# Maaz77/Head-Pose-Estimation-Model

Hardware: AMD Instinct MI355X
Metric: images/sec (train+infer) on 96×96 feature maps; yaw/pitch/roll MAE vs ref (higher is better)
Workload: dtype fp32; 1 GPU; Model-96 create_model(num_filters=360, dropout=0, l2=0.1) training, legacy Adam lr 2.8e-4, 96x96 feature maps (configs[3] per GPU: 512 images per rank); global_batch=512, per_gpu_batch=512, positions_per_image=9216, channels=96, parallelism=dp1

## Files before the change

### head-pose-estimation-model_amd/csrc/hpe_mlp2.hip

```cpp
#include <hip/hip_runtime.h>
#include <stdint.h>
#include <stdlib.h>
#include <type_traits>

#include "hpe_common.h"
#include "hpe_dev.h"

#ifdef MLP2_BIG
#define MLP2_NS mlp2_big
#define MLP2_BIG_OBJ 1
#else
#define MLP2_NS mlp2_small
#define MLP2_BIG_OBJ 0
#endif
#define MLP2_BIG_ROWS (1 << 15)
namespace MLP2_NS {

#define MLP2_MAXW 12
#ifndef MLP2_BAR1_SKIP
#define MLP2_BAR1_SKIP 1
#endif
#ifndef MLP2_W88
#define MLP2_W88 2
#endif
// ... 134 lines not shown
}
__device__ __forceinline__ constexpr int a1_row(int g) { return 68 * (g ^ ((g >> 1) & 4)); }
#define MLP2_X_LIMIT (65520.f / SPLIT_C)
template <int KH>
__device__ __forceinline__ bool presplit_tile(const float* xs, _Float16* xf, int tid, int NT) {
  bool out = false;
  for (int i = tid; i < 32 * 12; i += NT) {
    const int r = i / 12, rem = i - r * 12, h = rem >= 6 ? 1 : 0, m0 = 8 * (rem - 6 * h);
    const float* s = xs + r * MLP2_XS + KH * h + m0;
    const f32x4 z = {0.f, 0.f, 0.f, 0.f};
    const f32x4 a = *(const f32x4*)(s), b = m0 + 4 < KH ? *(const f32x4*)(s + 4) : z;
    const f32x8 v = {a.x, a.y, a.z, a.w, b.x, b.y, b.z, b.w};
#pragma unroll
    for (int j = 0; j < 8; ++j) out |= !(fabsf(v[j]) < MLP2_X_LIMIT);
    const SplitD d8 = split_d8(v);
    _Float16* d = xf + img_row(r) * MLP2_FS + 48 * h + m0;
    *(h8*)(d) = d8.ch;
    *(h8*)(d + 32 * MLP2_FS) = d8.cl;
    *(h8*)(d + 64 * MLP2_FS) = d8.h;
  }
  return out;
}

__device__ __forceinline__ SplitW split_w8_mix(f32x8 v) {
  SplitW r;
  r.h = __builtin_convertvector(v, h8);
  f32x8 lo;
#pragma unroll
  for (int j = 0; j < 8; ++j) lo[j] = __builtin_fmaf((float)r.h[j], -SPLIT_C, v[j] * SPLIT_C);
  r.cl = __builtin_convertvector(lo, h8);
  return r;
}

template <int KH, int ACT1, bool DROP, int NWM, bool SPLIT, bool CONTIG = false>
__global__ void __launch_bounds__(NWM * 64) __attribute__((amdgpu_waves_per_eu(NWM == MLP2_MAXW || ACT1 < 0 ? 1 : MLP2_W88, 8))) mlp2_kernel(Args args) {
  static_assert(!CONTIG || (SPLIT && NWM == MLP2_MAXW), "CONTIG is an instantiation of the pre-split kernel");
  if (!SPLIT && args.guard && __hip_atomic_load(args.guard, __ATOMIC_RELAXED, __HIP_MEMORY_SCOPE_AGENT) != args.epoch) return;
#ifdef MLP2_STAMPS
  const uint64_t rt0 = __builtin_amdgcn_s_memrealtime();
#endif
  extern __shared__ __attribute__((aligned(16))) float lds[];
  constexpr int NKB = (2 * KH + 31) / 32;
  constexpr int T = 32;
  constexpr bool PRE = SPLIT && NWM == MLP2_MAXW;
  constexpr int NXB = PRE ? 1 : 2;
  constexpr bool LEAN = PRE && ACT1 >= 0;
  constexpr bool EXPK = PRE && ACT1 == ACT_TANH;
  constexpr bool PAD1 = true;
  constexpr int A1S = MLP2_A1W;
  constexpr int HS = NWM == MLP2_MAXW ? 4 : 3;
  const int* prog = args.prog;
  const int* o = prog + prog[H_OPS_OFF];
  const int mode = prog[H_MODE];
  const bool train = mode == MODE_TRAIN;
  const int Cin = o[O_K], F = o[O_N], NCB = o[O_MODE];
  const int wave = __builtin_amdgcn_readfirstlane(threadIdx.x >> 6);
  const int lane = threadIdx.x & 63, half = lane >> 5, l32 = lane & 31;
  const int NT = blockDim.x;
  const int n = wave * 32 + l32;
  const bool nok = n < F;
  const int NPR = NWM == MLP2_MAXW ? MLP2_MAXW : NCB;
  float* xbuf = lds;
  float* lbuf = xbuf + NXB * MLP2_XF;
  float* part = lbuf + 2 * MLP2_LAB;
  float* dz2 = part + NPR * T * 4;
  float* a1s = dz2 + T * 4;
  float* w2t = a1s + NCB * A1S;
  float* b2t = w2t + NCB * 128;
  float* hacc = b2t + 4;
  float* red = hacc + NCB * 64 * HS;
  float* colt = red + MLP2_RED;
  _Float16* xfb = (_Float16*)(colt + NCB * 128);
  constexpr bool DZ2P = PRE && MLP2_BIG_OBJ;
  constexpr int DZS = DZ2P ? 3 : 4;

  E2 e1 = {o[O_EACT], o[O_EDROP], (uint32_t)o[O_ETHR], __int_as_float(o[O_EKEEP])};
  E2 e2 = {o[O_AUX2], o[O_TBASE], (uint32_t)o[O_TCOUNT], __int_as_float(o[O_F0])};
  const float inv_keep1 = 1.f / e1.keep;
  const float* W1 = args.params + o[O_W];
  const float* W2 = args.params + o[O_AUX0];

  const int64_t nrows = args.nrows;
  const int64_t ntiles = (nrows + T - 1) / T;
  const int P = args.P;
  const bool labels = mode != MODE_FWD;
  const int S = gridDim.x * T, dq = S / P, dr = S - dq * P;
  TileImg ti;
// ... 78 lines not shown
  }
  if (threadIdx.x < 4) b2t[threadIdx.x] = (threadIdx.x < 3 && o_aux1 >= 0) ? b2r : 0.f;
  for (int i = threadIdx.x; i < NT * HS; i += NT) hacc[i] = 0.f;

  f32x16 dw[NKB];
#pragma unroll
  for (int s = 0; s < NKB; ++s) dw[s] = f32x16{};
  float dw2[3] = {0.f, 0.f, 0.f};
  float db1 = 0.f;

  const int NT3 = (NT / 3) * 3;

  for (int i = threadIdx.x; i < NXB * 32 * 16; i += NT) {
    const int r = i >> 4, c = Cin + (i & 15);
    if (c < 96) xbuf[r * MLP2_XS + c] = 0.f;
  }
  for (int i = NCB * T * 4 + threadIdx.x; i < NPR * T * 4; i += NT) part[i] = 0.f;
  __syncthreads();
  if constexpr (PRE) {
    asm volatile("s_waitcnt vmcnt(0)" ::: "memory");
    bar_lds();
    const bool xbad = presplit_tile<KH>(xbuf, xfb, threadIdx.x, NT);
    bad |= xbad && blockIdx.x < ntiles;
  }
  int buf = 0;
#ifdef MLP2_STAMPS
  uint32_t ph[9] = {};
  uint64_t tprev = __builtin_amdgcn_s_memtime();
  const uint64_t rt1 = __builtin_amdgcn_s_memrealtime();
#define STAMP(i) do { const uint64_t t_ = __builtin_amdgcn_s_memtime(); ph[i] += (uint32_t)(t_ - tprev); tprev = t_; } while (0)
#else
#define STAMP(i) do {} while (0)
#endif
  for (int tile = blockIdx.x; tile < (int)ntiles; tile += gridDim.x, buf ^= 1, ti.advance(dq, dr)) {
    const int tlane = PRE ? lane_now() : lane, thalf = tlane >> 5, tl32 = tlane & 31;
    const int tcol = wave * 32 + tl32;
    const bool tok = tcol < F;
    using tid_t = typename std::conditional<PRE, int, unsigned>::type;
    const tid_t ttid = PRE ? (tid_t)(wave * 64 + tlane) : (tid_t)threadIdx.x;
    const int64_t row0 = (int64_t)tile * T;
    const float* xs = xbuf + (PRE ? 0 : buf) * MLP2_XF;
    const float* lab = lbuf + buf * MLP2_LAB;
    if constexpr (!PRE) asm volatile("s_waitcnt vmcnt(0)" ::: "memory");
    STAMP(0);
    if (!(MLP2_BAR1_SKIP && PRE && tile != (int)blockIdx.x)) bar_lds();
    STAMP(1);
    if (tile + gridDim.x < ntiles) {
      TileImg tn = ti;
      tn.advance(dq, dr);
      if constexpr (CONTIG) {
        stage_contig(args, xbuf, lbuf + (buf ^ 1) * MLP2_LAB, xnext, (int64_t)(tile + gridDim.x) * T, tn,
                     wave, NCB, Cin, labels);
        xnext += xstep;
      } else {
        stage_tile<PRE && MLP2_BIG_OBJ>(args, xbuf + (PRE ? 0 : (buf ^ 1)) * MLP2_XF, lbuf + (buf ^ 1) * MLP2_LAB,
                   (int64_t)(tile + gridDim.x) * T, tn, wave, NCB, tlane, Cin, labels);
      }
    }

    STAMP(2);
    uint32_t dmask = 0;
    {
      const float* ap = xs + tl32 * MLP2_XS + thalf * KH;
      f32x16 acc = {};
      if constexpr (PRE) {
        const _Float16* fp = xfb + buf * MLP2_IMG + img_row(tl32) * MLP2_FS + 48 * thalf;
        auto frag = [&](int s) {
          return SplitD{*(const h8*)(fp + 8 * s), *(const h8*)(fp + 32 * MLP2_FS + 8 * s),
                        *(const h8*)(fp + 64 * MLP2_FS + 8 * s)};
        };
        SplitD xd = frag(0);
#pragma unroll
        for (int s = 0; s < 6; ++s) {
          SplitD xn = xd;
          if (s + 1 < 6) xn = frag(s + 1);
          __builtin_amdgcn_sched_barrier(0);
          acc = mfma3_dw(xd, wsp[s], acc);
          xd = xn;
        }
        STAMP(3);
      } else if constexpr (SPLIT) {
#pragma unroll
        for (int s = 0; s < 6; ++s) {
          const f32x4 a0 = *(const f32x4*)(ap + 8 * s), a1 = *(const f32x4*)(ap + 8 * s + 4);
          acc = mfma3_dw(split_d8(f32x8{a0.x, a0.y, a0.z, a0.w, a1.x, a1.y, a1.z, a1.w}), wsp[s], acc);
          __builtin_amdgcn_sched_barrier(0);
        }
        bad |= !(fabsf(sum16(acc)) <= 3.0e38f);
      } else {
        f32x4 an = *(const f32x4*)(ap);
#pragma unroll
        for (int m = 0; m < KH; m += 4) {
          const f32x4 a = an;
          if (m + 4 < KH) an = *(const f32x4*)(ap + m + 4);
          acc = __builtin_amdgcn_mfma_f32_32x32x2f32(a.x, wreg[m + 0], acc, 0, 0, 0);
          acc = __builtin_amdgcn_mfma_f32_32x32x2f32(a.y, wreg[m + 1], acc, 0, 0, 0);
          acc = __builtin_amdgcn_mfma_f32_32x32x2f32(a.z, wreg[m + 2], acc, 0, 0, 0);
          acc = __builtin_amdgcn_mfma_f32_32x32x2f32(a.w, wreg[m + 3], acc, 0, 0, 0);
          __builtin_amdgcn_sched_barrier(0);
        }
      }
      if (DROP) {
        if (CONTIG || P >= 32) {
          const bool k0 = drop_hash(args.seed, e1.drop, (uint64_t)(ti.img0 + args.img_off), tcol) >= e1.thr;
          const bool k1 = drop_hash(args.seed, e1.drop, (uint64_t)(ti.img0 + 1 + args.img_off), tcol) >= e1.thr;
#pragma unroll
          for (int g = 0; g < 16; ++g) {
            const int r = (g & 3) + 8 * (g >> 2) + 4 * thalf;
            dmask |= (ti.rem0 + r >= P ? k1 : k0) ? (1u << g) : 0u;
          }
        } else {
#pragma unroll
          for (int g = 0; g < 16; ++g) {
            const int r = (g & 3) + 8 * (g >> 2) + 4 * thalf;
            dmask |= drop_hash(args.seed, e1.drop, (uint64_t)(ti.of(r) + args.img_off), tcol) >= e1.thr
                         ? (1u << g) : 0u;
          }
        }
      }
      const f32x4 cs = *(const f32x4*)(colt + tcol * 4);
#pragma unroll
      for (int g = 0; g < 16; ++g) {
        float z;
        if constexpr (EXPK) {
          const float e = __builtin_amdgcn_exp2f(fmaf(acc[g], cs.x, cs.y));
          z = fmaf(-2.f, __builtin_amdgcn_rcpf(1.f + e), 1.f);
        } else {
          z = act1_f<ACT1, SPLIT>(e1.act, SPLIT ? fmaf(acc[g], cs.x, cs.y) : acc[g] + cs.y);
        }
        if (DROP) z = (dmask >> g) & 1u ? z * inv_keep1 : 0.f;
        acc[g] = LEAN || tok ? z : 0.f;
      }
#pragma unroll
      for (int g = 0; g < 16; ++g) a1s[wave * A1S + (PAD1 ? a1_row(g) : 64 * g) + tlane] = acc[g];
      __builtin_amdgcn_fence(__ATOMIC_RELEASE, "wavefront");
      __builtin_amdgcn_wave_barrier();
      __builtin_amdgcn_fence(__ATOMIC_ACQUIRE, "wavefront");
      {
        const int r = tl32, hh = (r >> 2) & 1, gr = (r & 3) + 4 * (r >> 3);
        const float* ar = a1s + wave * A1S + (PAD1 ? a1_row(gr) : 64 * gr) + hh * 32 + 16 * thalf;
        const float* wr = w2t + (wave * 32 + 16 * thalf) * 4;
        float s0 = 0.f, s1 = 0.f, s2 = 0.f;
#pragma unroll
        for (int i = 0; i < 16; i += 4) {
          const f32x4 av = *(const f32x4*)(ar + i);
#pragma unroll
          for (int e = 0; e < 4; ++e) {
            const f32x4 w = *(const f32x4*)(wr + (i + e) * 4);
            s0 = fmaf(av[e], w.x, s0);
            s1 = fmaf(av[e], w.y, s1);
            s2 = fmaf(av[e], w.z, s2);
          }
        }
        if constexpr (PRE) {
          s0 += xor32_now(s0, tlane);
          s1 += xor32_now(s1, tlane);
          s2 += xor32_now(s2, tlane);
        } else {
          s0 += __shfl_xor(s0, 32, 64);
          s1 += __shfl_xor(s1, 32, 64);
          s2 += __shfl_xor(s2, 32, 64);
        }
        if (thalf == 0) *(f32x4*)(part + (wave * T + r) * 4) = f32x4{s0, s1, s2, 0.f};
      }
    }
    STAMP(4);
    if constexpr (PRE) asm volatile("s_waitcnt vmcnt(0)" ::: "memory");
    bar_lds();
    STAMP(5);
    if constexpr (PRE) {
      if (wave >= 2 && tile + gridDim.x < ntiles)
        bad |= presplit_tile<KH>(xbuf, xfb + (buf ^ 1) * MLP2_IMG, ttid - 128, NT - 128);
    }

    auto head_item = [&](int it) {
      const int r = it / 3, j = it - r * 3;
      const int64_t R = row0 + r;
      float z = b2t[j];
      float pv[MLP2_MAXW];
#pragma unroll
      for (int w = 0; w < MLP2_MAXW; ++w) pv[w] = NWM == MLP2_MAXW || w < NCB ? part[(w * T + r) * 4 + j] : 0.f;
      float lv = 0.f, ha0 = 0.f, ha1 = 0.f, ha2 = 0.f;
      if (mode != MODE_FWD) {
        lv = lab[r * 4 + j];
        ha0 = hacc[ttid * HS + 0];
        ha1 = hacc[ttid * HS + 1];
        ha2 = hacc[ttid * HS + 2];
      }
#pragma unroll
      for (int w = 0; w < MLP2_MAXW; ++w) z += pv[w];
      const bool d2 = ACT1 < 0 || __builtin_expect(e2.drop >= 0, 0);
      int64_t img = 0;
      bool k2 = true;
      if (d2) {
        img = ti.of<CONTIG>(r) + args.img_off;
        if (ACT1 >= 0) k2 = drop_hash(args.seed, e2.drop, (uint64_t)img, j) >= e2.thr;
      }
      const float p = ACT1 >= 0 ? (d2 ? (k2 ? z / e2.keep : 0.f) : z) : e_fwd(e2, args.seed, img, j, z);
      if (mode == MODE_FWD) {
        if (R < nrows) args.y[R * 3 + j] = p;
      } else {
        float g = 0.f;
        if (R < nrows) {
          const float err = p - lv;
          ha0 = fmaf(err, err, ha0);
          ha1 += fabsf(err);
          g = SPLIT ? 2.f * err : 2.f * err * args.inv_count;
        }
        if (train) {
          g = ACT1 >= 0 ? (d2 ? (k2 ? g / e2.keep : 0.f) : g) : e_bwd(e2, args.seed, img, j, g, p);
          dz2[r * DZS + j] = g;
          ha2 += g;
        }
        hacc[ttid * HS + 0] = ha0;
        hacc[ttid * HS + 1] = ha1;
        hacc[ttid * HS + 2] = ha2;
      }
    };
    if constexpr (NWM == MLP2_MAXW) {
      if (ttid < T * 3) head_item(ttid);
    } else {
      for (int it = threadIdx.x; it < T * 3 && threadIdx.x < NT3; it += NT3) head_item(it);
    }
    STAMP(6);
    if constexpr (PRE) {
      asm volatile("s_waitcnt vmcnt(0)" ::: "memory");
      bar_lds();
      STAMP(7);
      if (!train) continue;
    } else {
      if (!train) continue;
      bar_lds();
    }

    STAMP(8);
    {
      const f32x4 w2r = *(const f32x4*)(w2t + tcol * 4);
      const float s2 = colt[tcol * 4 + 2];
      const f32x4 w2v = PRE ? f32x4{w2r.x * s2, w2r.y * s2, w2r.z * s2, 0.f} : w2r;
      auto dz_row = [&](int g, float dx, float dy, float dz) {
        const float a = a1s[wave * A1S + (PAD1 ? a1_row(g) : 64 * g) + tlane];
        const float da = PRE ? fmaf(dz, w2v.z, fmaf(dx, w2v.x, dy * w2v.y))
                             : dx * w2v.x + dy * w2v.y + dz * w2v.z;
        float gz, av = a;
        if (DROP) {
          gz = (dmask >> g) & 1u ? da * inv_keep1 : 0.f;
          av = a * e1.keep;
        } else {
          gz = da;
        }
        {
#pragma clang fp contract(off)
          gz = LEAN || tok ? gz * act1_g<ACT1>(e1.act, av) : 0.f;
          db1 += gz;
        }
        dw2[0] = fmaf(a, dx, dw2[0]);
        dw2[1] = fmaf(a, dy, dw2[1]);
        dw2[2] = fmaf(a, dz, dw2[2]);
        return gz;
      };
      auto dz_of = [&](int g) {
        const int r = (g & 3) + 8 * (g >> 2) + 4 * thalf;
        const f32x4 d = *(const f32x4*)(dz2 + r * 4);
        return dz_row(g, d.x, d.y, d.z);
      };
      auto dz_step = [&](int s) {
        f32x8 dv;
#pragma unroll
        for (int k2 = 0; k2 < 2; ++k2) {
          const float* dp = dz2 + (8 * (2 * s + k2) + 4 * thalf) * 3;
          const f32x4 t0 = *(const f32x4*)(dp), t1 = *(const f32x4*)(dp + 4), t2 = *(const f32x4*)(dp + 8);
          const float t[12] = {t0.x, t0.y, t0.z, t0.w, t1.x, t1.y, t1.z, t1.w, t2.x, t2.y, t2.z, t2.w};
#pragma unroll
          for (int q = 0; q < 4; ++q) dv[4 * k2 + q] = dz_row(8 * s + 4 * k2 + q, t[3 * q], t[3 * q + 1], t[3 * q + 2]);
        }
        return dv;
      };
      if constexpr (PRE) {
        const int tc = (tl32 & 16) + 4 * (tl32 & 3);
        const _Float16* th = xfb + buf * MLP2_IMG + img_row(4 * thalf + ((tl32 >> 2) & 3)) * MLP2_FS;
        auto xt_of = [&](int s, int kb) {
          const _Float16* q = th + 16 * s * MLP2_FS + img_pos<KH>(32 * kb + tc);
          return SplitD{tr_read8(q), tr_read8(q + 32 * MLP2_FS), tr_read8(q + 64 * MLP2_FS)};
        };
        f32x8 dv0, dv1;
        if constexpr (DZ2P) dv0 = dz_step(0);
        else {
#pragma unroll
          for (int j = 0; j < 8; ++j) dv0[j] = dz_of(j);
        }
        const SplitW d0 = split_w8_mix(dv0);
        __builtin_amdgcn_sched_barrier(0);
#pragma unroll
        for (int kb = 0; kb < NKB; ++kb) dw[kb] = mfma3_dw(xt_of(0, kb), d0, dw[kb]);
        if constexpr (DZ2P) dv1 = dz_step(1);
        else {
#pragma unroll
          for (int j = 0; j < 8; ++j) dv1[j] = dz_of(8 + j);
        }
        __builtin_amdgcn_sched_barrier(0);
        const SplitW d1 = split_w8_mix(dv1);
#pragma unroll
        for (int kb = 0; kb < NKB; ++kb) dw[kb] = mfma3_dw(xt_of(1, kb), d1, dw[kb]);
      } else if constexpr (SPLIT) {
#pragma unroll
        for (int s = 0; s < 2; ++s) {
          f32x8 dv;
#pragma unroll
          for (int j = 0; j < 8; ++j) {
            dv[j] = dz_of(8 * s + j);
            if ((j & 3) == 3) __builtin_amdgcn_sched_barrier(0);
          }
          const SplitW dsp = split_w8(dv * s2);
#pragma unroll
          for (int kb = 0; kb < NKB; ++kb) {
            const float* xp = xs + (4 * thalf) * MLP2_XS + kb * 32 + tl32;
            f32x8 xv;
#pragma unroll
            for (int j = 0; j < 8; ++j) xv[j] = xp[(16 * s + 8 * (j >> 2) + (j & 3)) * MLP2_XS];
            dw[kb] = mfma3_dw(split_d8(xv), dsp, dw[kb]);
            __builtin_amdgcn_sched_barrier(0);
          }
        }
      } else {
        float dz1[16];
#pragma unroll
        for (int g = 0; g < 16; ++g) {
          dz1[g] = dz_of(g);
          if ((g & 3) == 3) __builtin_amdgcn_sched_barrier(0);
        }
#pragma unroll
        for (int kb = 0; kb < NKB; ++kb) {
          const float* xp = xs + (4 * thalf) * MLP2_XS + kb * 32 + tl32;
          f32x16 acc = dw[kb];
          auto xat = [&](int g) { return xp[((g & 3) + 8 * (g >> 2)) * MLP2_XS]; };
          float x0 = xat(0), x1 = xat(1);
#pragma unroll
          for (int g = 0; g < 16; ++g) {
            const float xv = x0;
            x0 = x1;
            if (g + 2 < 16) x1 = xat(g + 2);
            acc = __builtin_amdgcn_mfma_f32_32x32x2f32(xv, dz1[g], acc, 0, 0, 0);
            __builtin_amdgcn_sched_barrier(0);
          }
          dw[kb] = acc;
        }
      }
    }
  }

#ifdef MLP2_STAMPS
  const uint64_t rt2 = __builtin_amdgcn_s_memrealtime();
  uint64_t rtA = 0, rtB = 0;
  if (PRE && blockIdx.x == 0 && lane == 0 && (wave == 0 || wave == 5))
    printf("STAMP w%d bwd+tail %u bar1 %u stage %u fwdmfma %u act+part %u bar2 %u head %u bar3 %u presplit %u\n", wave,
           ph[0], ph[1], ph[2], ph[3], ph[4], ph[5], ph[6], ph[7], ph[8]);
#endif
  const int flane = PRE ? lane_now() : lane, fhalf = flane >> 5;
  const int fcol = wave * 32 + (flane & 31);
  const bool fok = fcol < F;
  if (mode == MODE_FWD) {
    if (SPLIT && bad) __hip_atomic_store(args.guard, args.epoch, __ATOMIC_RELAXED, __HIP_MEMORY_SCOPE_AGENT);
    return;
  }
  const int slab = prog[H_SLAB];
  const int npt = prog[H_NPARAMS_TRAIN];
  float* ws = args.ws + (size_t)blockIdx.x * slab;
  const float sc = SPLIT ? args.inv_count : 1.f;
  const int oW = __builtin_amdgcn_readfirstlane(o[O_W]), oB = __builtin_amdgcn_readfirstlane(o[O_BIAS]);
  const int oA0 = __builtin_amdgcn_readfirstlane(o[O_AUX0]), oA1 = __builtin_amdgcn_readfirstlane(o[O_AUX1]);
  __syncthreads();
  const float s2f = colt[fcol * 4 + 2];
  if (train) {
    const float scw = SPLIT ? sc * (SPLIT_INV_C / s2f) : sc;
    float chk = 0.f;
#pragma unroll
    for (int kb = 0; kb < NKB; ++kb) {
      if (SPLIT) chk += sum16(dw[kb]);
#pragma unroll
      for (int g = 0; g < 16; ++g) {
        const int k = kb * 32 + (g & 3) + 8 * (g >> 2) + 4 * fhalf;
        if (k < Cin && fok) ws[oW + (size_t)k * F + fcol] = dw[kb][g] * scw;
      }
    }
    if (SPLIT) bad |= (!LEAN || fok) && !(fabsf(chk) <= 3.0e38f);
    const float tb = (db1 + __shfl_xor(db1, 32, 64)) * (PRE ? 1.f / s2f : 1.f);
    float t2[3];
#pragma unroll
// ... 356 lines not shown
#pragma unroll
      for (int g = 0; g < 16; ++g) {
        const int k = kb * 32 + (g & 3) + 8 * (g >> 2) + 4 * half;
        if (k < Cin && nok[u]) ws[oW + (size_t)k * F + n] = dw[u][kb][g] * scw;
      }
    }
    const float tb = db1[u] + __shfl_xor(db1[u], 32, 64);
    float t2[3];
#pragma unroll
    for (int j = 0; j < 3; ++j) t2[j] = dw2[u][j] + __shfl_xor(dw2[u][j], 32, 64);
    if (half == 0 && nok[u]) {
      if (o_bias >= 0) ws[o_bias + n] = tb * sc;
#pragma unroll
      for (int j = 0; j < 3; ++j) ws[oA0 + n * 3 + j] = t2[j] * sc;
    }
  }
  bad |= !(fabsf(chk) <= 3.0e38f);
#pragma unroll
  for (int j = 0; j < 3; ++j) {
    const float t = wave_sum(db2[j]);
    if (lane == 0 && o_aux1 >= 0) ws[o_aux1 + j] = t * sc;
  }
  if (bad) __hip_atomic_store(args.guard, args.epoch, __ATOMIC_RELAXED, __HIP_MEMORY_SCOPE_AGENT);
  const float ta = wave_sum(sse), tb = wave_sum(sae);
  if (lane == 0) {
    ws[npt] = ta;
    ws[npt + 1] = tb;
  }
}
#endif

typedef void (*mlp2_fn)(Args);

template <int KH, bool DROP, int NWM, bool SPLIT, bool CONTIG = false>
static mlp2_fn pick_act(int act, int act2) {
  if (act2 != ACT_LINEAR) return mlp2_kernel<KH, -1, DROP, NWM, SPLIT, CONTIG>;
  if (act == ACT_TANH) return mlp2_kernel<KH, ACT_TANH, DROP, NWM, SPLIT, CONTIG>;
  if (act == ACT_SOFTSIGN) return mlp2_kernel<KH, ACT_SOFTSIGN, DROP, NWM, SPLIT, CONTIG>;
  return mlp2_kernel<KH, -1, DROP, NWM, SPLIT, CONTIG>;
}

template <bool DROP, bool SPLIT>
static mlp2_fn pick_d(int kh, int act, int act2, int ncb, bool contig) {
  if (ncb <= 4) {
    if (kh == 44) return pick_act<44, DROP, 4, SPLIT>(act, act2);
    if (kh == 48) return pick_act<48, DROP, 4, SPLIT>(act, act2);
  }
  if constexpr (SPLIT) {
    if (contig && kh == 44) return pick_act<44, DROP, MLP2_MAXW, SPLIT, true>(act, act2);
    if (contig && kh == 48) return pick_act<48, DROP, MLP2_MAXW, SPLIT, true>(act, act2);
  }
  if (kh == 44) return pick_act<44, DROP, MLP2_MAXW, SPLIT>(act, act2);
  if (kh == 48) return pick_act<48, DROP, MLP2_MAXW, SPLIT>(act, act2);
  return nullptr;
}

static mlp2_fn pick(const int* w, bool split = false, bool contig = false) {
  const int* o = w + w[H_OPS_OFF];
  const int kh = ((o[O_K] + 7) & ~7) / 2, act = o[O_EACT], act2 = o[O_AUX2];
  if (split)
    return o[O_EDROP] >= 0 ? pick_d<true, true>(kh, act, act2, o[O_MODE], contig) : pick_d<false, true>(kh, act, act2, o[O_MODE], contig);
  return o[O_EDROP] >= 0 ? pick_d<true, false>(kh, act, act2, o[O_MODE], false) : pick_d<false, false>(kh, act, act2, o[O_MODE], false);
}

static void geom(const int* w, int& kh, int& rbw, int& ncb, int& lds_bytes, int& act, int& drop) {
  const int* o = w + w[H_OPS_OFF];
  act = o[O_EACT];
  drop = o[O_EDROP];
  const int cin = o[O_K];
  const int cp = (cin + 7) & ~7;
  kh = cp / 2;
  rbw = o[O_FLAGS];
  ncb = o[O_MODE];
  const int T = 32;
  const int npr = ncb > 4 ? MLP2_MAXW : ncb;
  const int rest = 2 * MLP2_LAB + npr * T * 4 + T * 4 + ncb * MLP2_A1W + ncb * 128 + 4 + ncb * 64 * (ncb > 4 ? 4 : 3) + MLP2_RED + ncb * 128;
  lds_bytes = (2 * MLP2_XF + rest) * 4;
  const int pre = (MLP2_XF + rest) * 4 + MLP2_PRE_HALVES * 2;
  if (ncb > 4 && pre > lds_bytes) lds_bytes = pre;
}

static int lds_split(const int* w) {
  int kh, rbw, ncb, lds, act, drop;
  geom(w, kh, rbw, ncb, lds, act, drop);
  return lds;
}

static int launch_k(mlp2_fn k, int nw, int lds, const Args& a, int grid, hipStream_t s) {
  hipFuncSetAttribute((const void*)k, hipFuncAttributeMaxDynamicSharedMemorySize, lds);
  hipLaunchKernelGGL(k, dim3(grid), dim3(nw * 64), lds, s, a);
  return hipGetLastError() == hipSuccess ? 0 : 2;
}

static bool split_only() {
  const char* e = getenv("HPE_SPLIT_ONLY");
// ... 105 lines not shown
```

Measured before the change: 202,000 images/sec.

## Add rotated software-pipelined schedule overlapping next-tile forward with backward MFMAs

Adds a ROT instantiation of the contiguous pre-split MLP2 kernel, selected for training when dropout is off. It rotates the tile loop so the next tile's forward MFMAs and activation work are split into slices and interleaved with the current tile's backward dW1 MFMAs. Staging is issued two tiles ahead, and sched_group_barrier is used to co-issue VALU work with MFMA. The goal is to hide the forward phase's latency and drop one barrier per tile, at the cost of more register pressure and a more complex, harder-to-verify schedule.

```diff
diff --git a/head-pose-estimation-model_amd/csrc/hpe_mlp2.hip b/head-pose-estimation-model_amd/csrc/hpe_mlp2.hip
--- a/head-pose-estimation-model_amd/csrc/hpe_mlp2.hip
+++ b/head-pose-estimation-model_amd/csrc/hpe_mlp2.hip
@@ -190,9 +190,39 @@
   return r;
 }
 
-template <int KH, int ACT1, bool DROP, int NWM, bool SPLIT, bool CONTIG = false>
+#ifndef MLP2_ROT_DZ1
+#define MLP2_ROT_DZ1 0
+#endif
+#ifndef MLP2_ROT_FENCE
+#define MLP2_ROT_FENCE 3
+#endif
+#ifndef MLP2_ROT_FPER
+#define MLP2_ROT_FPER 1
+#endif
+#ifndef MLP2_PH1_VALU
+#define MLP2_PH1_VALU 9
+#endif
+#ifndef MLP2_PH2_VALU
+#define MLP2_PH2_VALU 9
+#endif
+template <int N_MFMA, int N_VALU>
+__device__ __forceinline__ void coissue_groups() {
+#pragma unroll
+  for (int i = 0; i < N_MFMA; ++i) {
+    __builtin_amdgcn_sched_group_barrier(0x008, 1, 0);
+    __builtin_amdgcn_sched_group_barrier(0x002, N_VALU, 0);
+  }
+}
+
+__device__ __forceinline__ constexpr int frag_off(int i) { return i == 0 ? 32 * MLP2_FS : i == 1 ? 64 * MLP2_FS : 0; }
+__device__ __forceinline__ f32x16 mfma3_dw_1(int i, h8 d, const SplitW& w, f32x16 acc) {
+  return __builtin_amdgcn_mfma_f32_32x32x16_f16(d, i == 1 ? w.cl : w.h, acc, 0, 0, 0);
+}
+
+template <int KH, int ACT1, bool DROP, int NWM, bool SPLIT, bool CONTIG = false, bool ROT = false>
 __global__ void __launch_bounds__(NWM * 64) __attribute__((amdgpu_waves_per_eu(NWM == MLP2_MAXW || ACT1 < 0 ? 1 : MLP2_W88, 8))) mlp2_kernel(Args args) {
   static_assert(!CONTIG || (SPLIT && NWM == MLP2_MAXW), "CONTIG is an instantiation of the pre-split kernel");
+  static_assert(!ROT || CONTIG, "ROT is a schedule of the contiguous-rows instantiation");
   if (!SPLIT && args.guard && __hip_atomic_load(args.guard, __ATOMIC_RELAXED, __HIP_MEMORY_SCOPE_AGENT) != args.epoch) return;
 #ifdef MLP2_STAMPS
   const uint64_t rt0 = __builtin_amdgcn_s_memrealtime();
@@ -210,7 +240,7 @@
   const int* prog = args.prog;
   const int* o = prog + prog[H_OPS_OFF];
   const int mode = prog[H_MODE];
-  const bool train = mode == MODE_TRAIN;
+  const bool train = ROT || mode == MODE_TRAIN;
   const int Cin = o[O_K], F = o[O_N], NCB = o[O_MODE];
   const int wave = __builtin_amdgcn_readfirstlane(threadIdx.x >> 6);
   const int lane = threadIdx.x & 63, half = lane >> 5, l32 = lane & 31;
@@ -355,209 +385,120 @@
 #else
 #define STAMP(i) do {} while (0)
 #endif
-  for (int tile = blockIdx.x; tile < (int)ntiles; tile += gridDim.x, buf ^= 1, ti.advance(dq, dr)) {
-    const int tlane = PRE ? lane_now() : lane, thalf = tlane >> 5, tl32 = tlane & 31;
-    const int tcol = wave * 32 + tl32;
-    const bool tok = tcol < F;
-    using tid_t = typename std::conditional<PRE, int, unsigned>::type;
-    const tid_t ttid = PRE ? (tid_t)(wave * 64 + tlane) : (tid_t)threadIdx.x;
-    const int64_t row0 = (int64_t)tile * T;
-    const float* xs = xbuf + (PRE ? 0 : buf) * MLP2_XF;
-    const float* lab = lbuf + buf * MLP2_LAB;
-    if constexpr (!PRE) asm volatile("s_waitcnt vmcnt(0)" ::: "memory");
-    STAMP(0);
-    if (!(MLP2_BAR1_SKIP && PRE && tile != (int)blockIdx.x)) bar_lds();
-    STAMP(1);
-    if (tile + gridDim.x < ntiles) {
-      TileImg tn = ti;
-      tn.advance(dq, dr);
-      if constexpr (CONTIG) {
-        stage_contig(args, xbuf, lbuf + (buf ^ 1) * MLP2_LAB, xnext, (int64_t)(tile + gridDim.x) * T, tn,
-                     wave, NCB, Cin, labels);
-        xnext += xstep;
+  struct LaneC {
+    int lane, half, l32, col;
+    bool ok;
+  };
+  auto no_slice = [](int) {};
+  auto fwd_pre = [&](int b, const LaneC& c, auto&& slice) {
+    f32x16 acc = {};
+    if constexpr (ROT) {
+      const _Float16* fp = xfb + b * MLP2_IMG + img_row(c.l32) * MLP2_FS + 48 * c.half;
+      auto frag1 = [&](int i) { return *(const h8*)(fp + frag_off(i % 3) + 8 * (i / 3)); };
+      h8 xd = frag1(0);
+#pragma unroll
+      for (int i = 0; i < 18; ++i) {
+        h8 xn = xd;
+        if (i + 1 < 18) xn = frag1(i + 1);
+        acc = mfma3_dw_1(i % 3, xd, wsp[i / 3], acc);
+        slice(i);
+        xd = xn;
+      }
+    } else if constexpr (PRE) {
+      const _Float16* fp = xfb + b * MLP2_IMG + img_row(c.l32) * MLP2_FS + 48 * c.half;
+      auto frag = [&](int s) {
+        return SplitD{*(const h8*)(fp + 8 * s), *(const h8*)(fp + 32 * MLP2_FS + 8 * s),
+                      *(const h8*)(fp + 64 * MLP2_FS + 8 * s)};
+      };
+      SplitD xd = frag(0);
+#pragma unroll
+      for (int s = 0; s < 6; ++s) {
+        SplitD xn = xd;
+        if (s + 1 < 6) xn = frag(s + 1);
+        if constexpr (!ROT) __builtin_amdgcn_sched_barrier(0);
+        acc = mfma3_dw(xd, wsp[s], acc);
+        xd = xn;
+      }
+    }
+    return acc;
+  };
+  auto act_park = [&](f32x16 acc, const TileImg& tix, const LaneC& c, auto&& slice) {
+    uint32_t dmask = 0;
+    if (DROP) {
+      if (CONTIG || P >= 32) {
+        const bool k0 = drop_hash(args.seed, e1.drop, (uint64_t)(tix.img0 + args.img_off), c.col) >= e1.thr;
+        const bool k1 = drop_hash(args.seed, e1.drop, (uint64_t)(tix.img0 + 1 + args.img_off), c.col) >= e1.thr;
+#pragma unroll
+        for (int g = 0; g < 16; ++g) {
+          const int r = (g & 3) + 8 * (g >> 2) + 4 * c.half;
+          dmask |= (tix.rem0 + r >= P ? k1 : k0) ? (1u << g) : 0u;
+        }
       } else {
-        stage_tile<PRE && MLP2_BIG_OBJ>(args, xbuf + (PRE ? 0 : (buf ^ 1)) * MLP2_XF, lbuf + (buf ^ 1) * MLP2_LAB,
-                   (int64_t)(tile + gridDim.x) * T, tn, wave, NCB, tlane, Cin, labels);
-      }
-    }
-
-    STAMP(2);
-    uint32_t dmask = 0;
+#pragma unroll
+        for (int g = 0; g < 16; ++g) {
+          const int r = (g & 3) + 8 * (g >> 2) + 4 * c.half;
+          dmask |= drop_hash(args.seed, e1.drop, (uint64_t)(tix.of(r) + args.img_off), c.col) >= e1.thr
+                       ? (1u << g) : 0u;
+        }
+      }
+    }
+    const f32x4 cs = *(const f32x4*)(colt + c.col * 4);
+#pragma unroll
+    for (int g = 0; g < 16; ++g) {
+      float z;
+      if constexpr (EXPK) {
+        const float e = __builtin_amdgcn_exp2f(fmaf(acc[g], cs.x, cs.y));
+        z = fmaf(-2.f, __builtin_amdgcn_rcpf(1.f + e), 1.f);
+      } else {
+        z = act1_f<ACT1, SPLIT>(e1.act, SPLIT ? fmaf(acc[g], cs.x, cs.y) : acc[g] + cs.y);
+      }
+      if (DROP) z = (dmask >> g) & 1u ? z * inv_keep1 : 0.f;
+      acc[g] = LEAN || c.ok ? z : 0.f;
+      if (g & 1) slice(g >> 1);
+    }
+#pragma unroll
+    for (int g = 0; g < 16; ++g) a1s[wave * A1S + (PAD1 ? a1_row(g) : 64 * g) + c.lane] = acc[g];
+    __builtin_amdgcn_fence(__ATOMIC_RELEASE, "wavefront");
+    __builtin_amdgcn_wave_barrier();
+    __builtin_amdgcn_fence(__ATOMIC_ACQUIRE, "wavefront");
     {
-      const float* ap = xs + tl32 * MLP2_XS + thalf * KH;
-      f32x16 acc = {};
+      const int r = c.l32, hh = (r >> 2) & 1, gr = (r & 3) + 4 * (r >> 3);
+      const float* ar = a1s + wave * A1S + (PAD1 ? a1_row(gr) : 64 * gr) + hh * 32 + 16 * c.half;
+      const float* wr = w2t + (wave * 32 + 16 * c.half) * 4;
+      float s0 = 0.f, s1 = 0.f, s2 = 0.f;
+#pragma unroll
+      for (int i = 0; i < 16; i += 4) {
+        const f32x4 av = *(const f32x4*)(ar + i);
+#pragma unroll
+        for (int e = 0; e < 4; ++e) {
+          const f32x4 w = *(const f32x4*)(wr + (i + e) * 4);
+          s0 = fmaf(av[e], w.x, s0);
+          s1 = fmaf(av[e], w.y, s1);
+          s2 = fmaf(av[e], w.z, s2);
+          if (e & 1) slice(8 + ((i + e) >> 1));
+        }
+      }
       if constexpr (PRE) {
-        const _Float16* fp = xfb + buf * MLP2_IMG + img_row(tl32) * MLP2_FS + 48 * thalf;
-        auto frag = [&](int s) {
-          return SplitD{*(const h8*)(fp + 8 * s), *(const h8*)(fp + 32 * MLP2_FS + 8 * s),
-                        *(const h8*)(fp + 64 * MLP2_FS + 8 * s)};
-        };
-        SplitD xd = frag(0);
-#pragma unroll
-        for (int s = 0; s < 6; ++s) {
-          SplitD xn = xd;
-          if (s + 1 < 6) xn = frag(s + 1);
-          __builtin_amdgcn_sched_barrier(0);
-          acc = mfma3_dw(xd, wsp[s], acc);
-          xd = xn;
-        }
-        STAMP(3);
-      } else if constexpr (SPLIT) {
-#pragma unroll
-        for (int s = 0; s < 6; ++s) {
-          const f32x4 a0 = *(const f32x4*)(ap + 8 * s), a1 = *(const f32x4*)(ap + 8 * s + 4);
-          acc = mfma3_dw(split_d8(f32x8{a0.x, a0.y, a0.z, a0.w, a1.x, a1.y, a1.z, a1.w}), wsp[s], acc);
-          __builtin_amdgcn_sched_barrier(0);
-        }
-        bad |= !(fabsf(sum16(acc)) <= 3.0e38f);
+        s0 += xor32_now(s0, c.lane);
+        slice(16);
+        s1 += xor32_now(s1, c.lane);
+        s2 += xor32_now(s2, c.lane);
       } else {
-        f32x4 an = *(const f32x4*)(ap);
-#pragma unroll
-        for (int m = 0; m < KH; m += 4) {
-          const f32x4 a = an;
-          if (m + 4 < KH) an = *(const f32x4*)(ap + m + 4);
-          acc = __builtin_amdgcn_mfma_f32_32x32x2f32(a.x, wreg[m + 0], acc, 0, 0, 0);
-          acc = __builtin_amdgcn_mfma_f32_32x32x2f32(a.y, wreg[m + 1], acc, 0, 0, 0);
-          acc = __builtin_amdgcn_mfma_f32_32x32x2f32(a.z, wreg[m + 2], acc, 0, 0, 0);
-          acc = __builtin_amdgcn_mfma_f32_32x32x2f32(a.w, wreg[m + 3], acc, 0, 0, 0);
-          __builtin_amdgcn_sched_barrier(0);
-        }
-      }
-      if (DROP) {
-        if (CONTIG || P >= 32) {
-          const bool k0 = drop_hash(args.seed, e1.drop, (uint64_t)(ti.img0 + args.img_off), tcol) >= e1.thr;
-          const bool k1 = drop_hash(args.seed, e1.drop, (uint64_t)(ti.img0 + 1 + args.img_off), tcol) >= e1.thr;
-#pragma unroll
-          for (int g = 0; g < 16; ++g) {
-            const int r = (g & 3) + 8 * (g >> 2) + 4 * thalf;
-            dmask |= (ti.rem0 + r >= P ? k1 : k0) ? (1u << g) : 0u;
-          }
-        } else {
-#pragma unroll
-          for (int g = 0; g < 16; ++g) {
-            const int r = (g & 3) + 8 * (g >> 2) + 4 * thalf;
-            dmask |= drop_hash(args.seed, e1.drop, (uint64_t)(ti.of(r) + args.img_off), tcol) >= e1.thr
-                         ? (1u << g) : 0u;
-          }
-        }
-      }
-      const f32x4 cs = *(const f32x4*)(colt + tcol * 4);
-#pragma unroll
-      for (int g = 0; g < 16; ++g) {
-        float z;
-        if constexpr (EXPK) {
-          const float e = __builtin_amdgcn_exp2f(fmaf(acc[g], cs.x, cs.y));
-          z = fmaf(-2.f, __builtin_amdgcn_rcpf(1.f + e), 1.f);
-        } else {
-          z = act1_f<ACT1, SPLIT>(e1.act, SPLIT ? fmaf(acc[g], cs.x, cs.y) : acc[g] + cs.y);
-        }
-        if (DROP) z = (dmask >> g) & 1u ? z * inv_keep1 : 0.f;
-        acc[g] = LEAN || tok ? z : 0.f;
-      }
-#pragma unroll
-      for (int g = 0; g < 16; ++g) a1s[wave * A1S + (PAD1 ? a1_row(g) : 64 * g) + tlane] = acc[g];
-      __builtin_amdgcn_fence(__ATOMIC_RELEASE, "wavefront");
-      __builtin_amdgcn_wave_barrier();
-      __builtin_amdgcn_fence(__ATOMIC_ACQUIRE, "wavefront");
-      {
-        const int r = tl32, hh = (r >> 2) & 1, gr = (r & 3) + 4 * (r >> 3);
-        const float* ar = a1s + wave * A1S + (PAD1 ? a1_row(gr) : 64 * gr) + hh * 32 + 16 * thalf;
-        const float* wr = w2t + (wave * 32 + 16 * thalf) * 4;
-        float s0 = 0.f, s1 = 0.f, s2 = 0.f;
-#pragma unroll
-        for (int i = 0; i < 16; i += 4) {
-          const f32x4 av = *(const f32x4*)(ar + i);
-#pragma unroll
-          for (int e = 0; e < 4; ++e) {
-            const f32x4 w = *(const f32x4*)(wr + (i + e) * 4);
-            s0 = fmaf(av[e], w.x, s0);
-            s1 = fmaf(av[e], w.y, s1);
-            s2 = fmaf(av[e], w.z, s2);
-          }
-        }
-        if constexpr (PRE) {
-          s0 += xor32_now(s0, tlane);
-          s1 += xor32_now(s1, tlane);
-          s2 += xor32_now(s2, tlane);
-        } else {
-          s0 += __shfl_xor(s0, 32, 64);
-          s1 += __shfl_xor(s1, 32, 64);
-          s2 += __shfl_xor(s2, 32, 64);
-        }
-        if (thalf == 0) *(f32x4*)(part + (wave * T + r) * 4) = f32x4{s0, s1, s2, 0.f};
-      }
-    }
-    STAMP(4);
-    if constexpr (PRE) asm volatile("s_waitcnt vmcnt(0)" ::: "memory");
-    bar_lds();
-    STAMP(5);
-    if constexpr (PRE) {
-      if (wave >= 2 && tile + gridDim.x < ntiles)
-        bad |= presplit_tile<KH>(xbuf, xfb + (buf ^ 1) * MLP2_IMG, ttid - 128, NT - 128);
-    }
-
-    auto head_item = [&](int it) {
-      const int r = it / 3, j = it - r * 3;
-      const int64_t R = row0 + r;
-      float z = b2t[j];
-      float pv[MLP2_MAXW];
-#pragma unroll
-      for (int w = 0; w < MLP2_MAXW; ++w) pv[w] = NWM == MLP2_MAXW || w < NCB ? part[(w * T + r) * 4 + j] : 0.f;
-      float lv = 0.f, ha0 = 0.f, ha1 = 0.f, ha2 = 0.f;
-      if (mode != MODE_FWD) {
-        lv = lab[r * 4 + j];
-        ha0 = hacc[ttid * HS + 0];
-        ha1 = hacc[ttid * HS + 1];
-        ha2 = hacc[ttid * HS + 2];
-      }
-#pragma unroll
-      for (int w = 0; w < MLP2_MAXW; ++w) z += pv[w];
-      const bool d2 = ACT1 < 0 || __builtin_expect(e2.drop >= 0, 0);
-      int64_t img = 0;
-      bool k2 = true;
-      if (d2) {
-        img = ti.of<CONTIG>(r) + args.img_off;
-        if (ACT1 >= 0) k2 = drop_hash(args.seed, e2.drop, (uint64_t)img, j) >= e2.thr;
-      }
-      const float p = ACT1 >= 0 ? (d2 ? (k2 ? z / e2.keep : 0.f) : z) : e_fwd(e2, args.seed, img, j, z);
-      if (mode == MODE_FWD) {
-        if (R < nrows) args.y[R * 3 + j] = p;
-      } else {
-        float g = 0.f;
-        if (R < nrows) {
-          const float err = p - lv;
-          ha0 = fmaf(err, err, ha0);
-          ha1 += fabsf(err);
-          g = SPLIT ? 2.f * err : 2.f * err * args.inv_count;
-        }
-        if (train) {
-          g = ACT1 >= 0 ? (d2 ? (k2 ? g / e2.keep : 0.f) : g) : e_bwd(e2, args.seed, img, j, g, p);
-          dz2[r * DZS + j] = g;
-          ha2 += g;
-        }
-        hacc[ttid * HS + 0] = ha0;
-        hacc[ttid * HS + 1] = ha1;
-        hacc[ttid * HS + 2] = ha2;
-      }
-    };
-    if constexpr (NWM == MLP2_MAXW) {
-      if (ttid < T * 3) head_item(ttid);
-    } else {
-      for (int it = threadIdx.x; it < T * 3 && threadIdx.x < NT3; it += NT3) head_item(it);
-    }
-    STAMP(6);
-    if constexpr (PRE) {
-      asm volatile("s_waitcnt vmcnt(0)" ::: "memory");
-      bar_lds();
-      STAMP(7);
-      if (!train) continue;
-    } else {
-      if (!train) continue;
-      bar_lds();
-    }
-
-    STAMP(8);
-    {
+        s0 += __shfl_xor(s0, 32, 64);
+        s1 += __shfl_xor(s1, 32, 64);
+        s2 += __shfl_xor(s2, 32, 64);
+      }
+      slice(17);
+      if (c.half == 0) *(f32x4*)(part + (wave * T + r) * 4) = f32x4{s0, s1, s2, 0.f};
+    }
+    return dmask;
+  };
+  uint32_t dmask = 0;
+  int tlane = 0, thalf = 0, tl32 = 0, tcol = 0;
+  bool tok = false;
+  LaneC lc = {};
+  const float* xs = xbuf;
+  auto backward = [&](auto more_c, int tile) {
       const f32x4 w2r = *(const f32x4*)(w2t + tcol * 4);
       const float s2 = colt[tcol * 4 + 2];
       const f32x4 w2v = PRE ? f32x4{w2r.x * s2, w2r.y * s2, w2r.z * s2, 0.f} : w2r;
@@ -587,16 +528,17 @@
         const f32x4 d = *(const f32x4*)(dz2 + r * 4);
         return dz_row(g, d.x, d.y, d.z);
       };
+      auto dz_half = [&](int s, int k2, f32x8& dv) {
+        const float* dp = dz2 + (8 * (2 * s + k2) + 4 * thalf) * 3;
+        const f32x4 t0 = *(const f32x4*)(dp), t1 = *(const f32x4*)(dp + 4), t2 = *(const f32x4*)(dp + 8);
+        const float t[12] = {t0.x, t0.y, t0.z, t0.w, t1.x, t1.y, t1.z, t1.w, t2.x, t2.y, t2.z, t2.w};
+#pragma unroll
+        for (int q = 0; q < 4; ++q) dv[4 * k2 + q] = dz_row(8 * s + 4 * k2 + q, t[3 * q], t[3 * q + 1], t[3 * q + 2]);
+      };
       auto dz_step = [&](int s) {
         f32x8 dv;
 #pragma unroll
-        for (int k2 = 0; k2 < 2; ++k2) {
-          const float* dp = dz2 + (8 * (2 * s + k2) + 4 * thalf) * 3;
-          const f32x4 t0 = *(const f32x4*)(dp), t1 = *(const f32x4*)(dp + 4), t2 = *(const f32x4*)(dp + 8);
-          const float t[12] = {t0.x, t0.y, t0.z, t0.w, t1.x, t1.y, t1.z, t1.w, t2.x, t2.y, t2.z, t2.w};
-#pragma unroll
-          for (int q = 0; q < 4; ++q) dv[4 * k2 + q] = dz_row(8 * s + 4 * k2 + q, t[3 * q], t[3 * q + 1], t[3 * q + 2]);
-        }
+        for (int k2 = 0; k2 < 2; ++k2) dz_half(s, k2, dv);
         return dv;
       };
       if constexpr (PRE) {
@@ -606,6 +548,64 @@
           const _Float16* q = th + 16 * s * MLP2_FS + img_pos<KH>(32 * kb + tc);
           return SplitD{tr_read8(q), tr_read8(q + 32 * MLP2_FS), tr_read8(q + 64 * MLP2_FS)};
         };
+        if constexpr (ROT) {
+          static_assert(!ROT || DZ2P, "ROT is a schedule of the big object's pre-split kernel");
+          if constexpr (decltype(more_c)::value) {
+            TileImg tn = ti;
+            tn.advance(dq, dr);
+            if (tile + 2 * gridDim.x < ntiles) {
+              TileImg tn2 = tn;
+              tn2.advance(dq, dr);
+              stage_contig(args, xbuf, lbuf + buf * MLP2_LAB, xnext, (int64_t)(tile + 2 * gridDim.x) * T, tn2,
+                           wave, NCB, Cin, labels);
+              xnext += xstep;
+            }
+            static_assert(!ROT || NKB == 3, "18 dW1 MFMAs per tile");
+            f32x8 dv0, dv1;
+            SplitW d0;
+            f32x4 t0, t1, t2;
+            auto xt1 = [&](int k) {
+              return tr_read8(th + 16 * (k / 9) * MLP2_FS + img_pos<KH>(32 * ((k % 9) / 3) + tc) + frag_off(k % 3));
+            };
+            auto pin_sums = [&] { asm volatile("" : "+v"(dw2[0]), "+v"(dw2[1]), "+v"(dw2[2]), "+v"(db1)); };
+            __builtin_amdgcn_sched_barrier(0);
+            const f32x16 accn = fwd_pre(buf ^ 1, lc, [&](int i) {
+              if (i == (MLP2_ROT_DZ1 ? 8 : 16)) d0 = split_w8_mix(dv0);
+              else if (MLP2_ROT_DZ1 ? i < 17 : !(i & 1)) {
+                const int g = MLP2_ROT_DZ1 ? (i < 8 ? i : i - 1) : i >> 1, q = g & 3;
+                if (q == 0) {
+                  const float* dp = dz2 + (8 * (g >> 2) + 4 * thalf) * 3;
+                  t0 = *(const f32x4*)(dp), t1 = *(const f32x4*)(dp + 4), t2 = *(const f32x4*)(dp + 8);
+                }
+                const float t[12] = {t0.x, t0.y, t0.z, t0.w, t1.x, t1.y, t1.z, t1.w, t2.x, t2.y, t2.z, t2.w};
+                (g < 8 ? dv0 : dv1)[g & 7] = dz_row(g, t[3 * q], t[3 * q + 1], t[3 * q + 2]);
+                pin_sums();
+              }
+              coissue_groups<1, MLP2_PH1_VALU>();
+              if (MLP2_ROT_FENCE & (1 << (i % MLP2_ROT_FPER == MLP2_ROT_FPER - 1))) __builtin_amdgcn_sched_barrier(0);
+            });
+            if (!MLP2_ROT_DZ1) {
+              dz_half(1, 0, dv1);
+              dz_half(1, 1, dv1);
+              pin_sums();
+            }
+            const SplitW d1 = split_w8_mix(dv1);
+            h8 xt = xt1(0);
+            __builtin_amdgcn_sched_barrier(0);
+            STAMP(3);
+            dmask = act_park(accn, tn, lc, [&](int k) {
+              h8 xn = xt;
+              if (k + 1 < 18) xn = xt1(k + 1);
+              const int kb = (k % 9) / 3;
+              dw[kb] = mfma3_dw_1(k % 3, xt, k < 9 ? d0 : d1, dw[kb]);
+              xt = xn;
+              coissue_groups<1, MLP2_PH2_VALU>();
+              if (MLP2_ROT_FENCE & (1 << (k % MLP2_ROT_FPER == MLP2_ROT_FPER - 1))) __builtin_amdgcn_sched_barrier(0);
+            });
+            STAMP(4);
+            return;
+          }
+        }
         f32x8 dv0, dv1;
         if constexpr (DZ2P) dv0 = dz_step(0);
         else {
@@ -669,14 +669,163 @@
           dw[kb] = acc;
         }
       }
-    }
-  }
+  };
+  if constexpr (ROT) {
+    if (blockIdx.x < ntiles) {
+      bar_lds();
+      if (blockIdx.x + gridDim.x < ntiles) {
+        TileImg tn = ti;
+        tn.advance(dq, dr);
+        stage_contig(args, xbuf, lbuf + MLP2_LAB, xnext, (int64_t)(blockIdx.x + gridDim.x) * T, tn, wave, NCB, Cin, labels);
+        xnext += xstep;
+      }
+      const int l = lane_now();
+      const LaneC c0 = {l, l >> 5, l & 31, wave * 32 + (l & 31), wave * 32 + (l & 31) < F};
+      dmask = act_park(fwd_pre(0, c0, no_slice), ti, c0, no_slice);
+    }
+  }
+  int tile = blockIdx.x;
+  auto run_tiles = [&](auto last_c) {
+    constexpr bool LAST = decltype(last_c)::value;
+    for (; LAST ? tile < (int)ntiles : tile + (int)gridDim.x < (int)ntiles; tile += gridDim.x, buf ^= 1, ti.advance(dq, dr)) {
+      tlane = PRE ? lane_now() : lane, thalf = tlane >> 5, tl32 = tlane & 31;
+      tcol = wave * 32 + tl32;
+      tok = tcol < F;
+      lc = {tlane, thalf, tl32, tcol, tok};
+      using tid_t = typename std::conditional<PRE, int, unsigned>::type;
+      const tid_t ttid = PRE ? (tid_t)(wave * 64 + tlane) : (tid_t)threadIdx.x;
+      const int64_t row0 = (int64_t)tile * T;
+      xs = xbuf + (PRE ? 0 : buf) * MLP2_XF;
+      const float* lab = lbuf + buf * MLP2_LAB;
+      if constexpr (!PRE) asm volatile("s_waitcnt vmcnt(0)" ::: "memory");
+      STAMP(0);
+      if (!ROT && !(MLP2_BAR1_SKIP && PRE && tile != (int)blockIdx.x)) bar_lds();
+      STAMP(1);
+      if (!ROT && tile + gridDim.x < ntiles) {
+        TileImg tn = ti;
+        tn.advance(dq, dr);
+        if constexpr (CONTIG) {
+          stage_contig(args, xbuf, lbuf + (buf ^ 1) * MLP2_LAB, xnext, (int64_t)(tile + gridDim.x) * T, tn,
+                       wave, NCB, Cin, labels);
+          xnext += xstep;
+        } else {
+          stage_tile<PRE && MLP2_BIG_OBJ>(args, xbuf + (PRE ? 0 : (buf ^ 1)) * MLP2_XF, lbuf + (buf ^ 1) * MLP2_LAB,
+                     (int64_t)(tile + gridDim.x) * T, tn, wave, NCB, tlane, Cin, labels);
+        }
+      }
+
+      STAMP(2);
+      if constexpr (!ROT) {
+        const float* ap = xs + tl32 * MLP2_XS + thalf * KH;
+        f32x16 acc = {};
+        if constexpr (PRE) {
+          acc = fwd_pre(buf, lc, no_slice);
+          STAMP(3);
+        } else if constexpr (SPLIT) {
+#pragma unroll
+          for (int s = 0; s < 6; ++s) {
+            const f32x4 a0 = *(const f32x4*)(ap + 8 * s), a1 = *(const f32x4*)(ap + 8 * s + 4);
+            acc = mfma3_dw(split_d8(f32x8{a0.x, a0.y, a0.z, a0.w, a1.x, a1.y, a1.z, a1.w}), wsp[s], acc);
+            __builtin_amdgcn_sched_barrier(0);
+          }
+          bad |= !(fabsf(sum16(acc)) <= 3.0e38f);
+        } else {
+          f32x4 an = *(const f32x4*)(ap);
+#pragma unroll
+          for (int m = 0; m < KH; m += 4) {
+            const f32x4 a = an;
+            if (m + 4 < KH) an = *(const f32x4*)(ap + m + 4);
+            acc = __builtin_amdgcn_mfma_f32_32x32x2f32(a.x, wreg[m + 0], acc, 0, 0, 0);
+            acc = __builtin_amdgcn_mfma_f32_32x32x2f32(a.y, wreg[m + 1], acc, 0, 0, 0);
+            acc = __builtin_amdgcn_mfma_f32_32x32x2f32(a.z, wreg[m + 2], acc, 0, 0, 0);
+            acc = __builtin_amdgcn_mfma_f32_32x32x2f32(a.w, wreg[m + 3], acc, 0, 0, 0);
+            __builtin_amdgcn_sched_barrier(0);
+          }
+        }
+        dmask = act_park(acc, ti, lc, no_slice);
+      }
+      STAMP(4);
+      if constexpr (PRE) asm volatile("s_waitcnt vmcnt(0)" ::: "memory");
+      bar_lds();
+      STAMP(5);
+      if constexpr (PRE) {
+        if (wave >= 2 && tile + gridDim.x < ntiles)
+          bad |= presplit_tile<KH>(xbuf, xfb + (buf ^ 1) * MLP2_IMG, ttid - 128, NT - 128);
+      }
+
+      auto head_item = [&](int it) {
+        const int r = it / 3, j = it - r * 3;
+        const int64_t R = row0 + r;
+        float z = b2t[j];
+        float pv[MLP2_MAXW];
+#pragma unroll
+        for (int w = 0; w < MLP2_MAXW; ++w) pv[w] = NWM == MLP2_MAXW || w < NCB ? part[(w * T + r) * 4 + j] : 0.f;
+        float lv = 0.f, ha0 = 0.f, ha1 = 0.f, ha2 = 0.f;
+        if (mode != MODE_FWD) {
+          lv = lab[r * 4 + j];
+          ha0 = hacc[ttid * HS + 0];
+          ha1 = hacc[ttid * HS + 1];
+          ha2 = hacc[ttid * HS + 2];
+        }
+#pragma unroll
+        for (int w = 0; w < MLP2_MAXW; ++w) z += pv[w];
+        const bool d2 = ACT1 < 0 || __builtin_expect(e2.drop >= 0, 0);
+        int64_t img = 0;
+        bool k2 = true;
+        if (d2) {
+          img = ti.of<CONTIG>(r) + args.img_off;
+          if (ACT1 >= 0) k2 = drop_hash(args.seed, e2.drop, (uint64_t)img, j) >= e2.thr;
+        }
+        const float p = ACT1 >= 0 ? (d2 ? (k2 ? z / e2.keep : 0.f) : z) : e_fwd(e2, args.seed, img, j, z);
+        if (mode == MODE_FWD) {
+          if (R < nrows) args.y[R * 3 + j] = p;
+        } else {
+          float g = 0.f;
+          if (R < nrows) {
+            const float err = p - lv;
+            ha0 = fmaf(err, err, ha0);
+            ha1 += fabsf(err);
+            g = SPLIT ? 2.f * err : 2.f * err * args.inv_count;
+          }
+          if (train) {
+            g = ACT1 >= 0 ? (d2 ? (k2 ? g / e2.keep : 0.f) : g) : e_bwd(e2, args.seed, img, j, g, p);
+            dz2[r * DZS + j] = g;
+            ha2 += g;
+          }
+          hacc[ttid * HS + 0] = ha0;
+          hacc[ttid * HS + 1] = ha1;
+          hacc[ttid * HS + 2] = ha2;
+        }
+      };
+      if constexpr (NWM == MLP2_MAXW) {
+        if (ttid < T * 3) head_item(ttid);
+      } else {
+        for (int it = threadIdx.x; it < T * 3 && threadIdx.x < NT3; it += NT3) head_item(it);
+      }
+      STAMP(6);
+      if constexpr (PRE) {
+        asm volatile("s_waitcnt vmcnt(0)" ::: "memory");
+        bar_lds();
+        STAMP(7);
+        if (!train) continue;
+      } else {
+        if (!train) continue;
+        bar_lds();
+      }
+
+      STAMP(8);
+      backward(std::integral_constant<bool, ROT && !LAST>{}, tile);
+    }
+  };
+  if constexpr (ROT) run_tiles(std::false_type{});
+  run_tiles(std::true_type{});
 
 #ifdef MLP2_STAMPS
   const uint64_t rt2 = __builtin_amdgcn_s_memrealtime();
   uint64_t rtA = 0, rtB = 0;
   if (PRE && blockIdx.x == 0 && lane == 0 && (wave == 0 || wave == 5))
-    printf("STAMP w%d bwd+tail %u bar1 %u stage %u fwdmfma %u act+part %u bar2 %u head %u bar3 %u presplit %u\n", wave,
+    printf(ROT ? "STAMP w%d rot last-bwd+tail %u - %u - %u phase1 %u stage+phase2 %u bar2 %u head %u bar3 %u presplit %u\n"
+               : "STAMP w%d bwd+tail %u bar1 %u stage %u fwdmfma %u act+part %u bar2 %u head %u bar3 %u presplit %u\n", wave,
            ph[0], ph[1], ph[2], ph[3], ph[4], ph[5], ph[6], ph[7], ph[8]);
 #endif
   const int flane = PRE ? lane_now() : lane, fhalf = flane >> 5;
@@ -1099,20 +1248,24 @@
 
 typedef void (*mlp2_fn)(Args);
 
-template <int KH, bool DROP, int NWM, bool SPLIT, bool CONTIG = false>
+template <int KH, bool DROP, int NWM, bool SPLIT, bool CONTIG = false, bool ROT = false>
 static mlp2_fn pick_act(int act, int act2) {
   if (act2 != ACT_LINEAR) return mlp2_kernel<KH, -1, DROP, NWM, SPLIT, CONTIG>;
-  if (act == ACT_TANH) return mlp2_kernel<KH, ACT_TANH, DROP, NWM, SPLIT, CONTIG>;
-  if (act == ACT_SOFTSIGN) return mlp2_kernel<KH, ACT_SOFTSIGN, DROP, NWM, SPLIT, CONTIG>;
+  if (act == ACT_TANH) return mlp2_kernel<KH, ACT_TANH, DROP, NWM, SPLIT, CONTIG, ROT>;
+  if (act == ACT_SOFTSIGN) return mlp2_kernel<KH, ACT_SOFTSIGN, DROP, NWM, SPLIT, CONTIG, ROT>;
   return mlp2_kernel<KH, -1, DROP, NWM, SPLIT, CONTIG>;
 }
 
 template <bool DROP, bool SPLIT>
-static mlp2_fn pick_d(int kh, int act, int act2, int ncb, bool contig) {
+static mlp2_fn pick_d(int kh, int act, int act2, int ncb, bool contig, bool rot) {
   if (ncb <= 4) {
     if (kh == 44) return pick_act<44, DROP, 4, SPLIT>(act, act2);
     if (kh == 48) return pick_act<48, DROP, 4, SPLIT>(act, act2);
   }
+  if constexpr (SPLIT && MLP2_BIG_OBJ && !DROP) {
+    if (contig && rot && kh == 44) return pick_act<44, DROP, MLP2_MAXW, SPLIT, true, true>(act, act2);
+    if (contig && rot && kh == 48) return pick_act<48, DROP, MLP2_MAXW, SPLIT, true, true>(act, act2);
+  }
   if constexpr (SPLIT) {
     if (contig && kh == 44) return pick_act<44, DROP, MLP2_MAXW, SPLIT, true>(act, act2);
     if (contig && kh == 48) return pick_act<48, DROP, MLP2_MAXW, SPLIT, true>(act, act2);
@@ -1125,9 +1278,10 @@
 static mlp2_fn pick(const int* w, bool split = false, bool contig = false) {
   const int* o = w + w[H_OPS_OFF];
   const int kh = ((o[O_K] + 7) & ~7) / 2, act = o[O_EACT], act2 = o[O_AUX2];
+  const bool rot = w[H_MODE] == MODE_TRAIN;
   if (split)
-    return o[O_EDROP] >= 0 ? pick_d<true, true>(kh, act, act2, o[O_MODE], contig) : pick_d<false, true>(kh, act, act2, o[O_MODE], contig);
-  return o[O_EDROP] >= 0 ? pick_d<true, false>(kh, act, act2, o[O_MODE], false) : pick_d<false, false>(kh, act, act2, o[O_MODE], false);
+    return o[O_EDROP] >= 0 ? pick_d<true, true>(kh, act, act2, o[O_MODE], contig, rot) : pick_d<false, true>(kh, act, act2, o[O_MODE], contig, rot);
+  return o[O_EDROP] >= 0 ? pick_d<true, false>(kh, act, act2, o[O_MODE], false, false) : pick_d<false, false>(kh, act, act2, o[O_MODE], false, false);
 }
 
 static void geom(const int* w, int& kh, int& rbw, int& ncb, int& lds_bytes, int& act, int& drop) {
```

Result: slower. 196,700 images/sec (-2.6%).
